# mabdullahsoyturk/Torch-Sputnik

Measured on AMD Instinct MI355X. Metric: SpMM effective GFLOP/s (2*nnz*N/t), M=N=K=4096 fp32, density 0.1, higher is better.
Workload: dtype f32

## Files before the change

torch_sputnik_amd/csrc/gen_spmm_flat.py:

```python
#!/usr/bin/env python3
import argparse

_ap = argparse.ArgumentParser()
_ap.add_argument("--mode", default="entry", choices=["entry", "group"])
_ap.add_argument("--layout", default="straight", choices=["straight", "diagonal"])
_ap.add_argument("out", nargs="?")
ARGS = _ap.parse_args()
GROUP = ARGS.mode == "group"

BK = 32
BK_SHIFT = 5
ROW_BYTES = 2048
ROW_SHIFT = 11
WIN_BYTES = 144
NSTRIP = 4
NPIECES = 4
ROWSTEP = 8

V_LANE, V_STAGE, V_PLAN, V_ROWS = "v0", "v1", "v2", "v3"
CUR_OFF, CUR_VAL = 4, 5
NXT_OFF, NXT_VAL, NXT_ROWS = 6, 7, 8
NN_OFF, NN_VAL, NN_ROWS = 10, 11, 12
PAIR = [16, 18, 20, 22]
VALT = [16, 18]
V_ADDR = 20
STRIP = [32, 40, 48, 56]
ACC = 64

S_STREAM, S_VALUES, S_CINFO, S_DENSE = "s[36:37]", "s[38:39]", "s[40:41]", "s[42:43]"
S_PITCH, S_KMAX, S_NCHUNKS, S_ROW0, S_LDS0, S_DEBUG = "s44", "s45", "s46", "s47", "s48", "s49"
S_REM, S_C, S_CIOFF, S_MINE, S_SB, S_NSW = "s50", "s51", "s56", "s57", "s76", "s77"
S_CI = ["s52", "s53", "s54", "s55"]
S_RET, S_BND = "s[58:59]", "s[60:61]"
S_ROWS = [62, 63, 64, 65]
S_IDX = [66, 67, 68, 69]
S_COLS = "s78"
S_T = ["s70", "s71", "s72", "s73", "s74", "s75"]

out = []


def emit(line):
    out.append(line)


def label(name):
    return f".L_{name}_%="


def strip_reads(ring, addr):
    s = STRIP[ring]
    emit(f"ds_read_b128 v[{s}:{s + 3}], v{addr}")
    emit(f"ds_read_b128 v[{s + 4}:{s + 7}], v{addr} offset:1024")


def fmas(src_pair, op_sel, ring):
    s = STRIP[ring]
    for q in range(4):
        emit(f"v_pk_fma_f32 v[{ACC + 2 * q}:{ACC + 2 * q + 1}], v[{src_pair}:{src_pair + 1}], "
             f"v[{s + 2 * q}:{s + 2 * q + 1}], v[{ACC + 2 * q}:{ACC + 2 * q + 1}] {op_sel}")


def entry_fma_stage(ring, lgkm):
    emit(f"s_waitcnt lgkmcnt({lgkm})")
    emit(f"s_set_gpr_idx_on s{S_IDX[ring]}, 0xc")
    fmas(PAIR[ring], "op_sel:[1,0,0] op_sel_hi:[1,1,1]", ring)
    emit("s_set_gpr_idx_off")


def entry_slot(slot):
    ring = slot % NSTRIP
    p = PAIR[ring]
    emit(f"{label(f'E_{slot}')}:")
    emit(f"s_sub_u32 {S_REM}, {S_REM}, 1")
    emit(f"s_cbranch_scc1 {label(f'bnd_{slot}')}")
    emit(f"v_mov_b64_dpp v[{p}:{p + 1}], v[{CUR_OFF}:{CUR_VAL}] row_newbcast:{slot} row_mask:0xf bank_mask:0xf")
    emit(f"s_bfe_u32 s{S_IDX[ring]}, s{S_ROWS[slot // 4]}, {hex(8 * (slot % 4) | (7 << 16))}")
    emit(f"v_add_u32 v{p}, v{p}, {V_LANE}")
    strip_reads(ring, p)
    entry_fma_stage((ring + 1) % NSTRIP, 2 * (NSTRIP - 1))


def group_entry_body(ring, slot):
    t = VALT[slot % 2]
    emit(f"v_mov_b32_dpp v{t}, v{CUR_VAL} row_newbcast:{slot} row_mask:0xf bank_mask:0xf")
    emit(f"s_bfe_u32 s{S_IDX[0]}, s{S_ROWS[slot // 4]}, {hex(8 * (slot % 4) | (7 << 16))}")
    emit(f"s_set_gpr_idx_on s{S_IDX[0]}, 0xc")
    fmas(t, "op_sel:[0,0,0] op_sel_hi:[0,1,1]", ring)
    emit("s_set_gpr_idx_off")


def group_start(ring, slot):
    emit(f"{label(f'N_{ring}_{slot}')}:")
    emit(f"s_sub_u32 {S_REM}, {S_REM}, 1")
    emit(f"s_cbranch_scc1 {label(f'bnd_{slot}')}")
    emit(f"v_mov_b32_dpp v{V_ADDR}, v{CUR_OFF} row_newbcast:{slot} row_mask:0xf bank_mask:0xf")
    emit(f"v_add_u32 v{V_ADDR}, v{V_ADDR}, {V_LANE}")
    strip_reads(ring, V_ADDR)
    emit(f"s_waitcnt lgkmcnt({2 * (NSTRIP - 1)})")


def first_groups():
    for i in range(NSTRIP - 1):
        emit(f"s_bfe_u32 {S_T[0]}, {S_COLS}, {hex(8 * i | (8 << 16))}")
        emit(f"s_lshl_b32 {S_T[0]}, {S_T[0]}, {ROW_SHIFT}")
        emit(f"v_add_u32 v{V_ADDR}, {S_T[0]}, {V_LANE}")
        strip_reads(i, V_ADDR)


def stage_chunk(chunk_sgpr):
    t_row, t_lds, t_r, t_lo, t_hi = S_T[1], S_T[2], S_T[3], S_T[4], S_T[5]
    emit(f"s_lshl_b32 {t_row}, {chunk_sgpr}, {BK_SHIFT}")
    emit(f"s_add_u32 {t_row}, {t_row}, {S_ROW0}")
    emit(f"s_and_b32 {t_lds}, {chunk_sgpr}, 1")
    emit(f"s_lshl_b32 {t_lds}, {t_lds}, 16")
    emit(f"s_add_u32 {t_lds}, {t_lds}, {S_LDS0}")
    for i in range(NPIECES):
        emit(f"s_add_u32 {t_r}, {t_row}, {ROWSTEP * i}")
        emit(f"s_min_u32 {t_r}, {t_r}, {S_KMAX}")
        emit(f"s_mul_hi_u32 {t_hi}, {t_r}, {S_PITCH}")
        emit(f"s_mul_i32 {t_lo}, {t_r}, {S_PITCH}")
        emit(f"s_add_u32 {t_lo}, {t_lo}, s42")
        emit(f"s_addc_u32 {t_hi}, {t_hi}, s43")
        emit(f"s_add_u32 m0, {t_lds}, {hex(ROWSTEP * i * ROW_BYTES)}")
        emit("s_nop 0")
        emit(f"global_load_lds_dwordx4 {V_STAGE}, s[{t_lo[1:]}:{t_hi[1:]}]")


def plan_load(off, rows):
    emit(f"global_load_dwordx2 v[{off}:{off + 1}], {V_PLAN}, {S_STREAM}")
    emit(f"global_load_dword v{rows}, {V_ROWS}, {S_STREAM}")
    emit(f"v_add_u32 {V_PLAN}, {hex(WIN_BYTES)}, {V_PLAN}")
    emit(f"v_add_u32 {V_ROWS}, {hex(WIN_BYTES)}, {V_ROWS}")


def gather(val):
    emit(f"global_load_dword v{val}, v{val}, {S_VALUES}")


def switch_window(tag):
    emit(f"s_cmp_lg_u32 {S_SB}, 0")
    emit(f"s_cbranch_scc1 {label('swc_' + tag)}")
    emit("s_waitcnt vmcnt(0)")
    emit(f"s_branch {label('swd_' + tag)}")
    emit(f"{label('swc_' + tag)}:")
    emit(f"s_waitcnt vmcnt({NPIECES})")
    emit(f"{label('swd_' + tag)}:")
    emit(f"s_mov_b32 {S_SB}, 0")
    emit(f"s_add_u32 {S_NSW}, {S_NSW}, 1")
    for i in range(4):
        emit(f"v_readlane_b32 s{S_ROWS[i]}, v{NXT_ROWS}, {i}")
    emit(f"v_bfe_u32 v{CUR_OFF}, v{NXT_OFF}, {8 if GROUP else 0}, 8")
    emit(f"v_mov_b32 v{CUR_VAL}, v{NXT_VAL}")
    emit(f"v_lshlrev_b32 v{CUR_OFF}, {ROW_SHIFT}, v{CUR_OFF}")
    emit(f"v_mov_b64 v[{NXT_OFF}:{NXT_VAL}], v[{NN_OFF}:{NN_VAL}]")
    emit(f"v_mov_b32 v{NXT_ROWS}, v{NN_ROWS}")
    emit(f"s_bitcmp1_b32 {S_DEBUG}, 3")
    emit(f"s_cbranch_scc1 {label('swskip_' + tag)}")
    gather(NXT_VAL)
    plan_load(NN_OFF, NN_ROWS)
    emit(f"{label('swskip_' + tag)}:")
    emit("s_nop 1")


def take_chunk_info():
    emit(f"s_mov_b32 {S_REM}, {S_CI[0] if GROUP else S_CI[3]}")
    if GROUP:
        emit(f"s_mov_b32 {S_COLS}, {S_CI[1]}")


def generate():
    emit("; ---- prologue ----")
    for r in list(range(ACC, ACC + 64)) + list(range(STRIP[0], STRIP[0] + 32)) + list(range(16, 24)):
        emit(f"v_mov_b32 v{r}, 0")
    for r in S_IDX:
        emit(f"s_mov_b32 s{r}, 0")
    emit(f"s_getpc_b64 {S_BND}")
    emit(f"{label('pc')}:")
    emit(f"s_add_u32 s60, s60, {label('boundary')}-{label('pc')}")
    emit("s_addc_u32 s61, s61, 0")
    plan_load(NXT_OFF, NXT_ROWS)
    plan_load(NN_OFF, NN_ROWS)
    emit("s_waitcnt vmcnt(2)")
    gather(NXT_VAL)
    emit(f"s_mov_b32 {S_T[0]}, 0")
    stage_chunk(S_T[0])
    emit(f"s_load_dwordx4 s[52:55], {S_CINFO}, 0x0")
    emit("s_waitcnt vmcnt(0) lgkmcnt(0)")
    emit("s_barrier")
    take_chunk_info()
    emit(f"s_load_dwordx4 s[52:55], {S_CINFO}, 0x10")
    emit(f"s_mov_b32 {S_CIOFF}, 32")
    emit(f"s_mov_b32 {S_C}, 0")
    emit(f"s_mov_b32 {S_NSW}, 0")
    emit(f"s_mov_b32 {S_SB}, 0")
    emit(f"s_mov_b32 {S_MINE}, 0")
    if GROUP:
        first_groups()
    emit(f"s_cmp_lt_u32 {S_NCHUNKS}, 2")
    emit(f"s_cbranch_scc1 {label('pro_nostage')}")
    emit(f"s_mov_b32 {S_T[0]}, 1")
    stage_chunk(S_T[0])
    emit(f"s_mov_b32 {S_SB}, 1")
    emit(f"s_mov_b32 {S_MINE}, 1")
    emit(f"{label('pro_nostage')}:")
    switch_window("pro")

    emit("; ---- main loop ----")
    if not GROUP:
        for slot in range(16):
            entry_slot(slot)
        switch_window("w")
        emit(f"s_branch {label('E_0')}")
    elif ARGS.layout == "straight":
        emit(f"s_branch {label(f'E_{NSTRIP - 1}_0')}")
        for ring in range(NSTRIP):
            for slot in range(16):
                emit(f"{label(f'E_{ring}_{slot}')}:")
                emit(f"s_bitcmp1_b32 s{S_ROWS[slot // 4]}, {8 * (slot % 4) + 7}")
                emit(f"s_cbranch_scc1 {label(f'N_{ring}_{slot}')}")
                emit(f"{label(f'B_{ring}_{slot}')}:")
                group_entry_body(ring, slot)
            switch_window(f"r{ring}")
            emit(f"s_branch {label(f'E_{ring}_0')}")
        emit("; ---- first entry of a column group ----")
        for ring in range(NSTRIP):
            for slot in range(16):
                group_start(ring, slot)
                emit(f"s_branch {label(f'B_{(ring + 1) % NSTRIP}_{slot}')}")
    else:
        emit(f"s_branch {label(f'E_{NSTRIP - 1}_0')}")
        for diag in range(NSTRIP):
            for slot in range(16):
                ring = (diag + slot) % NSTRIP
                emit(f"{label(f'E_{ring}_{slot}')}:")
                emit(f"s_bitcmp1_b32 s{S_ROWS[slot // 4]}, {8 * (slot % 4) + 7}")
                emit(f"s_cbranch_scc0 {label(f'B_{ring}_{slot}')}")
                group_start(ring, slot)
                emit(f"{label(f'B_{(ring + 1) % NSTRIP}_{slot}')}:")
                group_entry_body((ring + 1) % NSTRIP, slot)
            ring = (diag + 16) % NSTRIP
            switch_window(f"r{diag}")
            emit(f"s_branch {label(f'E_{ring}_0')}")

    emit("; ---- boundary stubs ----")
    for slot in range(16):
        emit(f"{label(f'bnd_{slot}')}:")
        emit(f"s_swappc_b64 {S_RET}, {S_BND}")
        if GROUP:
            emit(f"s_cbranch_scc1 {label('end')}")
            emit(f"s_branch {label(f'N_{NSTRIP - 1}_{slot}')}")
        else:
            emit(f"s_cbranch_scc1 {label(f'drain_{slot % NSTRIP}')}")
            emit(f"s_branch {label(f'E_{slot}')}")

    emit("; ---- boundary subroutine ----")
    emit(f"{label('boundary')}:")
    emit(f"s_bitcmp1_b32 {S_DEBUG}, 2")
    emit(f"s_cbranch_scc1 {label('bnodrain')}")
    emit("s_waitcnt lgkmcnt(0)")
    emit(f"{label('bnodrain')}:")
    emit(f"s_cmp_eq_u32 {S_MINE}, 0")
    emit(f"s_cbranch_scc1 {label('bvd')}")
    emit(f"s_bitcmp1_b32 {S_DEBUG}, 5")
    emit(f"s_cbranch_scc1 {label('bvd')}")
    for n in range(3):
        emit(f"s_cmp_eq_u32 {S_NSW}, {n}")
        emit(f"s_cbranch_scc1 {label(f'bv{n}')}")
    emit("s_waitcnt vmcnt(9)")
    emit(f"s_branch {label('bvd')}")
    for n in range(3):
        emit(f"{label(f'bv{n}')}:")
        emit(f"s_waitcnt vmcnt({3 * n})")
        if n < 2:
            emit(f"s_branch {label('bvd')}")
    emit(f"{label('bvd')}:")
    emit(f"s_bitcmp1_b32 {S_DEBUG}, 1")
    emit(f"s_cbranch_scc1 {label('bnobar')}")
    emit("s_barrier")
    emit(f"{label('bnobar')}:")
    emit(f"s_add_u32 {S_C}, {S_C}, 1")
    emit(f"s_cmp_eq_u32 {S_C}, {S_NCHUNKS}")
    emit(f"s_cbranch_scc1 {label('bret')}")
    take_chunk_info()
    emit(f"s_load_dwordx4 s[52:55], {S_CINFO}, {S_CIOFF}")
    emit(f"s_add_u32 {S_CIOFF}, {S_CIOFF}, 16")
    if GROUP:
        first_groups()
    emit(f"s_mov_b32 {S_NSW}, 0")
    emit(f"s_mov_b32 {S_MINE}, 0")
    emit(f"s_add_u32 {S_T[0]}, {S_C}, 1")
    emit(f"s_cmp_ge_u32 {S_T[0]}, {S_NCHUNKS}")
    emit(f"s_cbranch_scc1 {label('bnostage')}")
    emit(f"s_bitcmp1_b32 {S_DEBUG}, 0")
    emit(f"s_cbranch_scc1 {label('bnostage')}")
    stage_chunk(S_T[0])
    emit(f"s_add_u32 {S_SB}, {S_SB}, 1")
    emit(f"s_mov_b32 {S_MINE}, 1")
    emit(f"{label('bnostage')}:")
    emit(f"s_cmp_eq_u32 {S_C}, {S_NCHUNKS}")
    emit(f"{label('bret')}:")
    emit(f"s_setpc_b64 {S_RET}")

    if not GROUP:
        emit("; ---- drain: the three entries still in the pipeline ----")
        for ring in range(NSTRIP):
            emit(f"{label(f'drain_{ring}')}:")
            for j in range(1, NSTRIP):
                entry_fma_stage((ring + j) % NSTRIP, 2 * (NSTRIP - 1 - j))
            if ring < NSTRIP - 1:
                emit(f"s_branch {label('end')}")
    emit(f"{label('end')}:")
    emit("s_waitcnt vmcnt(0) lgkmcnt(0)")


def main():
    generate()
    text = "// GENERATED by gen_spmm_flat.py -- do not edit.\n" + "".join(
        f'"{line}\\n"\n' for line in out)
    if ARGS.out:
        with open(ARGS.out, "w") as f:
            f.write(text)
    else:
        print(text, end="")


if __name__ == "__main__":
    main()
```

torch_sputnik_amd/csrc/spmm_flat.hip:

```cpp
#include <algorithm>

#include "options.h"
#include "spmm_tiled_common.h"

namespace sputnik_hip {

namespace {

using namespace tiled;

constexpr int kBN = 512;
constexpr int kBK = 32;
constexpr int kWaves = 16;
constexpr int kRPW = 8;
constexpr int kBM = kWaves * kRPW;
constexpr int kAhead = 3;
constexpr int kDealPer = 256;
constexpr int kWindow = 16;
constexpr int kWindowBytes = 144;
constexpr int kTailWindows = 4;
constexpr int kMaxColumns = 65536;
constexpr unsigned kNewGroup = 0x80;


struct ChunkInfo {
  int groups;
  unsigned first_rows;
  unsigned unused;
  int entries;
};

__host__ __device__ inline size_t fill_tables_bytes(int nchunks) {
  return (sizeof(int) * (static_cast<size_t>(nchunks) * (kBK / 4 + 4) + 2 * kRPW + 2) + 15) / 16 * 16;
}
__device__ __forceinline__ int wave_sum(int v) {
#pragma unroll
  for (int o = 32; o > 0; o >>= 1) v += __shfl_xor(v, o);
  return v;
}
__device__ __forceinline__ int wave_inclusive_scan(int v, int lane) {
#pragma unroll
  for (int o = 1; o < 64; o <<= 1) {
    const int t = __shfl_up(v, o);
    if (lane >= o) v += t;
  }
  return v;
}

__global__ __launch_bounds__(kRPW * 64) void spmm_flat_fill_kernel(
    int m, int k, int slots, int nchunks, const int* __restrict__ row_indices,
    const int* __restrict__ row_offsets, const int* __restrict__ column_indices,
    int* __restrict__ row_ok, ChunkInfo* __restrict__ cinfo, int* __restrict__ gwin,
    unsigned char* __restrict__ stream, int stage_windows, int debug) {
  extern __shared__ unsigned lds[];
  constexpr int RPW = kRPW, BK = kBK, NT = RPW * 64;
  constexpr int WPC = BK / 4;
  constexpr int UN = 4;
  const int g = blockIdx.x, tid = threadIdx.x, lane = tid % 64, wave = tid / 64;
  const int groups = gridDim.x;
  unsigned* maskw = lds;
  int* ebase = reinterpret_cast<int*>(lds + nchunks * WPC);
  unsigned* nzmask = reinterpret_cast<unsigned*>(ebase + nchunks);
  unsigned* wprefix = nzmask + nchunks;
  int* scratch = reinterpret_cast<int*>(wprefix + 2 * nchunks);
  unsigned char* sbuf = reinterpret_cast<unsigned char*>(lds) + fill_tables_bytes(nchunks);

  for (int i = tid; i < nchunks * WPC; i += NT) maskw[i] = 0;
  const int slot = g * RPW + wave;
  const int entry = dealt_index(slot, slots, kDealPer);
  int p0 = 0, p1 = 0;
  if (entry < m) {
    const int row = row_indices[entry];
    p0 = row_offsets[row];
    p1 = row_offsets[row + 1];
  }
  int before = 0;
  for (int gp = tid; gp < g; gp += NT) {
    int rows[RPW], len = 0;
    int2 bounds[RPW];
#pragma unroll
    for (int r = 0; r < RPW; ++r) {
      const int e = dealt_index(gp * RPW + r, slots, kDealPer);
      rows[r] = e < m ? row_indices[e] : -1;
    }
#pragma unroll
    for (int r = 0; r < RPW; ++r) {
      typedef int int2_a4 __attribute__((ext_vector_type(2), aligned(4)));
      if (rows[r] >= 0) {
        const int2_a4 pair = *reinterpret_cast<const int2_a4*>(row_offsets + rows[r]);
        bounds[r] = make_int2(pair.x, pair.y);
      } else {
        bounds[r] = make_int2(0, 0);
      }
    }
#pragma unroll
    for (int r = 0; r < RPW; ++r) len += bounds[r].y - bounds[r].x;
    before += (len + kWindow - 1) / kWindow;
  }
  before = wave_sum(before);
  if (lane == 0) {
    scratch[wave] = before;
    scratch[RPW + wave] = p1 - p0;
  }
  if (tid == 0) scratch[2 * RPW] = 1;
  __syncthreads();
  int wbase = 0, total = 0;
#pragma unroll
  for (int r = 0; r < RPW; ++r) {
    wbase += scratch[r];
    total += scratch[RPW + r];
  }
  if (tid == 0) gwin[g] = wbase;
  unsigned char* my_stream = stream + static_cast<int64_t>(wbase) * kWindowBytes;
  const int windows = (total + kWindow - 1) / kWindow;

  bool ok = true;
  for (int base = p0; base < p1; base += 64 * UN) {
    int cur[UN], prev[UN];
#pragma unroll
    for (int u = 0; u < UN; ++u) {
      const int p = base + u * 64 + lane;
      cur[u] = p < p1 ? column_indices[p] : -2;
    }
    const int before_base = base > p0 ? column_indices[base - 1] : -1;
#pragma unroll
    for (int u = 0; u < UN; ++u) {
      const int up = __shfl_up(cur[u], 1);
      const int carry = u == 0 ? before_base : __shfl(cur[u == 0 ? 0 : u - 1], 63);
      prev[u] = lane == 0 ? carry : up;
    }
#pragma unroll
    for (int u = 0; u < UN; ++u) {
      if (cur[u] == -2) continue;
      if (cur[u] <= prev[u] || cur[u] >= k) ok = false;
      else atomicOr(&maskw[cur[u] >> 2], (1u << wave) << (8 * (cur[u] & 3)));
    }
  }
  const bool wave_ok = __builtin_amdgcn_ballot_w64(!ok) == 0;
  if (lane == 0) {
    row_ok[slot] = wave_ok ? 1 : 0;
    if (!wave_ok) scratch[2 * RPW] = 0;
  }
  __syncthreads();
  ChunkInfo* my_info = cinfo + static_cast<int64_t>(g) * (nchunks + 1);
  if (scratch[2 * RPW] == 0) {
    unsigned* w = reinterpret_cast<unsigned*>(my_stream);
    const int nwin = windows + (g == groups - 1 ? kTailWindows : 0);
    for (int i = tid; i < nwin * (kWindowBytes / 4); i += NT)
      w[i] = i % (kWindowBytes / 4) >= 32 ? 0x80808080u : 0u;
    for (int c = tid; c <= nchunks; c += NT) my_info[c] = ChunkInfo{0, 0u, 0u, 0};
    return;
  }

  if (debug & 0x100) return;
  for (int t0 = 0; t0 < nchunks * WPC; t0 += NT) {
    const int t = t0 + tid;
    const bool live = t < nchunks * WPC;
    const int c = t / WPC, i = t % WPC;
    const unsigned w = live ? maskw[t] : 0u;
    const int cnt = __popc(w);
    unsigned nz = 0u;
#pragma unroll
    for (int b = 0; b < 4; ++b)
      if ((w >> (8 * b)) & 0xffu) nz |= 1u << (4 * i + b);
    int incl = cnt;
#pragma unroll
    for (int o = 1; o < WPC; o <<= 1) {
      const int up = __shfl_up(incl, o, WPC);
      if (i >= o) incl += up;
    }
#pragma unroll
    for (int o = 1; o < WPC; o <<= 1) nz |= static_cast<unsigned>(__shfl_xor(static_cast<int>(nz), o, WPC));
    const int entries = __shfl(incl, WPC - 1, WPC);
    if (live) {
      reinterpret_cast<unsigned char*>(wprefix)[t] = static_cast<unsigned char>(incl - cnt);
      if (i == 0) {
        unsigned first = 0u, rest = nz;
        const int cgroups = __popc(nz);
#pragma unroll
        for (int q = 0; q < kAhead; ++q)
          if (rest) {
            first |= static_cast<unsigned>((c & 1) * BK + __ffs(rest) - 1) << (8 * q);
            rest &= rest - 1u;
          }
        ebase[c] = entries;
        nzmask[c] = nz;
        my_info[c] = ChunkInfo{cgroups, first, 0u, entries};
      }
    }
  }
  if (tid == 0) my_info[nchunks] = ChunkInfo{0, 0u, 0u, 0};
  __syncthreads();
  if (wave == 0) {
    int carry = 0;
    for (int c0 = 0; c0 < nchunks; c0 += 64) {
      const int c = c0 + lane;
      const int e = c < nchunks ? ebase[c] : 0;
      const int incl = wave_inclusive_scan(e, lane);
      if (c < nchunks) ebase[c] = carry + incl - e;
      carry += __shfl(incl, 63);
    }
  }
  __syncthreads();

  if (debug & 0x200) return;
  static_assert(WPC == 8, "two prefix words per chunk");
  const int nwin_out = windows + (g == groups - 1 ? kTailWindows : 0);
  const bool staged = nwin_out <= stage_windows && !(debug & 0x1000);
  unsigned char* const dst_stream = staged ? sbuf : my_stream;
  for (int base = p0; base < p1; base += 64 * UN) {
    int cols[UN];
#pragma unroll
    for (int u = 0; u < UN; ++u) {
      const int p = base + u * 64 + lane;
      cols[u] = p < p1 ? column_indices[p] : -1;
    }
#pragma unroll
    for (int u = 0; u < UN; ++u) {
      if (cols[u] < 0) continue;
      const int p = base + u * 64 + lane;
      const int col = cols[u], c = col / BK, j = col % BK;
      const unsigned w = maskw[c * WPC + j / 4];
      const int prefix = static_cast<int>((wprefix[2 * c + j / 16] >> (8 * ((j / 4) % 4))) & 0xffu) +
                         __popc(w & ((1u << (8 * (j & 3))) - 1u));
      const unsigned byte = (w >> (8 * (j & 3))) & 0xffu;
      const int own = __popc(byte & ((1u << wave) - 1u));
      const int pos = ebase[c] + prefix + own;
      unsigned rowbyte = wave * 8, tile_rows = static_cast<unsigned>((c & 1) * BK + j);
      if (own == 0) {
        rowbyte |= kNewGroup;
        unsigned ahead = j == BK - 1 ? 0u : nzmask[c] >> (j + 1);
        ahead &= ahead - 1u;
        ahead &= ahead - 1u;
        if (ahead) tile_rows |= static_cast<unsigned>((c & 1) * BK + j + __ffs(ahead)) << 8;
      }
      if (debug & 0x400) continue;
      unsigned char* block = dst_stream + static_cast<int64_t>(pos / kWindow) * kWindowBytes;
      const int e = pos % kWindow;
      *reinterpret_cast<uint2*>(block + 8 * e) = make_uint2(tile_rows, static_cast<unsigned>(p) * 4u);
      block[128 + e] = static_cast<unsigned char>(rowbyte);
    }
  }
  for (int pos = total + tid; pos < windows * kWindow; pos += NT) {
    unsigned char* block = dst_stream + static_cast<int64_t>(pos / kWindow) * kWindowBytes;
    *reinterpret_cast<uint2*>(block + 8 * (pos % kWindow)) = make_uint2(0u, 0u);
    block[128 + pos % kWindow] = static_cast<unsigned char>(kNewGroup);
  }
  if (g == groups - 1) {
    unsigned* w = reinterpret_cast<unsigned*>(dst_stream + static_cast<int64_t>(windows) * kWindowBytes);
    for (int i = tid; i < kTailWindows * (kWindowBytes / 4); i += NT)
      w[i] = i % (kWindowBytes / 4) >= 32 ? 0x80808080u : 0u;
  }
  if (staged) {
    __syncthreads();
    const uint4* src = reinterpret_cast<const uint4*>(sbuf);
    uint4* dst = reinterpret_cast<uint4*>(my_stream);
    for (int i = tid; i < nwin_out * (kWindowBytes / 16); i += NT) dst[i] = src[i];
  }
}

using v8f = float __attribute__((ext_vector_type(8)));

#define SPUTNIK_HIP_FLAT_ASM_OPERANDS                                                              \
      : "={v[64:71]}"(a0), "={v[72:79]}"(a1), "={v[80:87]}"(a2), "={v[88:95]}"(a3),                \
        "={v[96:103]}"(a4), "={v[104:111]}"(a5), "={v[112:119]}"(a6), "={v[120:127]}"(a7)          \
      : "{v0}"(lane_base), "{v1}"(stage_off), "{v2}"(plan_off), "{v3}"(rows_off),                  \
        "{s[36:37]}"(my_stream), "{s[38:39]}"(values), "{s[40:41]}"(my_info), "{s[42:43]}"(dense), \
        "{s44}"(pitch), "{s45}"(kmax), "{s46}"(nchunks), "{s47}"(row0), "{s48}"(lds0),             \
        "{s49}"(debug)                                                                             \
      : "memory", "m0", "scc", "v4", "v5", "v6", "v7", "v8", "v9", "v10", "v11", "v12", "v13",     \
        "v14", "v15", "v16", "v17", "v18", "v19", "v20", "v21", "v22", "v23", "v32", "v33", "v34", \
        "v35", "v36", "v37", "v38", "v39", "v40", "v41", "v42", "v43", "v44", "v45", "v46", "v47", \
        "v48", "v49", "v50", "v51", "v52", "v53", "v54", "v55", "v56", "v57", "v58", "v59", "v60", \
        "v61", "v62", "v63", "s50", "s51", "s52", "s53", "s54", "s55", "s56", "s57", "s58", "s59", \
        "s60", "s61", "s62", "s63", "s64", "s65", "s66", "s67", "s68", "s69", "s70", "s71", "s72", \
        "s73", "s74", "s75", "s76", "s77", "s78", "s79", "s80"

template <int LOOP>
__global__ __launch_bounds__(kWaves * 64) void spmm_flat_kernel(
    int m, int k, int n, int slots, int nchunks, int n_tiles, const int* __restrict__ row_indices,
    const float* __restrict__ values, int64_t values_stride, const ChunkInfo* __restrict__ cinfo,
    const int* __restrict__ gwin, const unsigned char* __restrict__ stream,
    const float* __restrict__ dense, int64_t dense_stride, float* __restrict__ out,
    int64_t out_stride, const int* __restrict__ row_ok, const int* __restrict__ row_offsets,
    const int* __restrict__ column_indices, int debug, Epilogue epi) {
  constexpr int RPW = kRPW, BM = kBM, BN = kBN, BK = kBK, VEC = 8;
  constexpr int PPR = VEC / 4;
  __shared__ float tile[2][BK * BN];

  const int lane = threadIdx.x % kWave;
  const int wave = __builtin_amdgcn_readfirstlane(threadIdx.x / kWave);

  const int bid = blockIdx.x;
  int ntile, mblock;
  int replica = blockIdx.y;
  const int xcd_cols = 1 << ((debug >> 13) & 3);
  if (xcd_cols > 1 && n_tiles == 8 && (gridDim.x / 8) % xcd_cols == 0) {
    const int xcd = bid % 8, i = bid / 8, col_groups = 8 / xcd_cols;
    ntile = (xcd % col_groups) * xcd_cols + i % xcd_cols;
    mblock = (xcd / col_groups) * ((gridDim.x / 8) / xcd_cols) + i / xcd_cols;
  } else if (n_tiles % 8 == 0) {
    const int per_xcd = n_tiles / 8;
    const int xcd = bid % 8, i = bid / 8;
    ntile = xcd * per_xcd + i % per_xcd;
    mblock = i / per_xcd;
  } else {
    const int work = xcd_local_index32();
    const int mblocks = gridDim.x / n_tiles;
    mblock = work % mblocks;
    ntile = (work / mblocks) % n_tiles;
    replica = work / (mblocks * n_tiles);
  }
  values += replica * values_stride;
  dense += replica * dense_stride;
  out += replica * out_stride;

  const int n0 = ntile * BN;
  const int slot0 = mblock * BM + wave * RPW;

  if (!block_rows_ok_wave(row_ok, mblock * BM, BM)) {
    for (int r = 0; r < RPW; ++r) {
      const int entry = dealt_index(slot0 + r, slots, kDealPer);
      if (entry >= m) continue;
      const int row = row_indices[entry];
#pragma unroll
      for (int h = 0; h < PPR; ++h) {
        if (n0 + h * 256 + lane * 4 >= n) continue;
        const int col = min(n0 + h * 256 + lane * 4, n - 4);
        const float4 acc4 = gather_row_strip(values, column_indices, row_offsets[row],
                                             row_offsets[row + 1], dense + col, n);
        *reinterpret_cast<float4*>(out + static_cast<int64_t>(row) * n + col) =
            apply_epilogue(acc4, epi, row);
      }
    }
    return;
  }

  const int group = slot0 / RPW;
  const unsigned char* my_stream =
      stream + static_cast<int64_t>(__builtin_amdgcn_readfirstlane(gwin[group])) * kWindowBytes;
  const ChunkInfo* my_info = cinfo + static_cast<int64_t>(group) * (nchunks + 1);
  const unsigned tile_lds = static_cast<unsigned>(reinterpret_cast<uintptr_t>(AS_LDS(&tile[0][0])));
  const unsigned lane_base = tile_lds + lane * 16;
  const unsigned stage_off =
      static_cast<unsigned>(min(n0 + (wave % PPR) * 256 + lane * 4, n - 4)) * 4u;
  const unsigned plan_off = (lane & 15) * 8, rows_off = 128 + (lane & 3) * 4;
  const int pitch = n * 4, kmax = k - 1, row0 = wave / PPR;
  const int lds0 = static_cast<int>(tile_lds) + (wave / PPR) * (BN * 4) + (wave % PPR) * 1024;

  v8f a0, a1, a2, a3, a4, a5, a6, a7;
  if constexpr (LOOP == 0) {
    asm volatile(
#include "spmm_flat_body_entry.inc"
        SPUTNIK_HIP_FLAT_ASM_OPERANDS);
  } else if constexpr (LOOP == 1) {
    asm volatile(
#include "spmm_flat_body_group_s.inc"
        SPUTNIK_HIP_FLAT_ASM_OPERANDS);
  } else {
    asm volatile(
#include "spmm_flat_body_group_d.inc"
        SPUTNIK_HIP_FLAT_ASM_OPERANDS);
  }

  const v8f acc[8] = {a0, a1, a2, a3, a4, a5, a6, a7};
#pragma unroll
  for (int r = 0; r < RPW; ++r) {
    const int entry = dealt_index(slot0 + r, slots, kDealPer);
    if (entry < m) {
      const int row = row_indices[entry];
#pragma unroll
      for (int h = 0; h < PPR; ++h)
        if (n0 + h * 256 + lane * 4 < n) {
          const int col = min(n0 + h * 256 + lane * 4, n - 4);
          const int f = r * VEC + 4 * h;
          *reinterpret_cast<float4*>(out + static_cast<int64_t>(row) * n + col) =
              apply_epilogue(make_float4(acc[f / 8][f % 8], acc[f / 8][f % 8 + 1],
                                         acc[f / 8][f % 8 + 2], acc[f / 8][f % 8 + 3]),
                             epi, row);
        }
    }
  }
}

struct FlatPlan {
  int slots, nchunks, n_tiles, groups;
  size_t row_ok_off, cinfo_off, gwin_off, stream_off, bytes;
};

FlatPlan make_flat_plan(int m, int k, int n, int nonzeros) {
  FlatPlan p;
  p.slots = ceil_div(m, kDealPer) * kDealPer;
  p.nchunks = ceil_div(k, kBK);
  p.n_tiles = ceil_div(n, kBN);
  p.groups = p.slots / kRPW;
  auto up = [](size_t v) { return (v + 255) / 256 * 256; };
  p.row_ok_off = 0;
  p.cinfo_off = row_ok_bytes(p.slots);
  p.gwin_off = up(p.cinfo_off + sizeof(ChunkInfo) * static_cast<size_t>(p.nchunks + 1) * p.groups);
  p.stream_off = up(p.gwin_off + sizeof(int) * static_cast<size_t>(p.groups));
  const size_t windows = static_cast<size_t>(nonzeros) / kWindow + p.groups + kTailWindows;
  p.bytes = up(p.stream_off + windows * kWindowBytes);
  return p;
}

int fill_stage_windows(int nchunks, int nonzeros, int groups) {
  const size_t tables = fill_tables_bytes(nchunks);
  if (tables + kWindowBytes > 64 * 1024) return 0;
  const int64_t room = static_cast<int64_t>((64 * 1024 - tables) / kWindowBytes);
  const int64_t want = (static_cast<int64_t>(nonzeros) / kWindow / groups) * 5 / 4 + kTailWindows + 2;
  return static_cast<int>(std::min(room, want));
}
size_t fill_lds_bytes(int nchunks, int stage_windows) {
  return fill_tables_bytes(nchunks) + static_cast<size_t>(stage_windows) * kWindowBytes;
}

int flat_mode(int m, int k, int nonzeros) {
  const int forced = options().spmm_sparse;
  if (forced >= 2 && forced <= 4) return forced - 2;
  const double d = static_cast<double>(nonzeros) / (static_cast<double>(m) * k);
  return d < 0.12 ? 0 : d < 0.36 ? 2 : 1;
}

}

static bool fill_lds_available(int k) {
  static const bool extended = [] {
    return hipFuncSetAttribute(reinterpret_cast<const void*>(spmm_flat_fill_kernel),
                               hipFuncAttributeMaxDynamicSharedMemorySize,
                               static_cast<int>(fill_lds_bytes(kMaxColumns / kBK, 0))) == hipSuccess;
  }();
  return extended || fill_lds_bytes(ceil_div(k, kBK), 0) <= 64 * 1024;
}

bool spmm_flat_applicable(int m, int k, int n, int nonzeros) {
  if (n < 4 || k < kBK || m < 64 || nonzeros < 16 * static_cast<int64_t>(m) ||
      nonzeros >= (1 << 29))
    return false;
  if (static_cast<int64_t>(ceil_div(n, kBN)) * kBN * 3 > static_cast<int64_t>(n) * 4) return false;
  return k <= kMaxColumns && m <= 16384 && fill_lds_available(k);
}

const char* spmm_flat_kernel_name(int m, int k, int nonzeros) {
  static const char* const names[] = {"spmm_flat_kernel<0>", "spmm_flat_kernel<1>", "spmm_flat_kernel<2>"};
  return names[flat_mode(m, k, nonzeros)];
}

int64_t spmm_flat_tiles(int m, int n) {
  return static_cast<int64_t>(ceil_div(m, kBM)) * ceil_div(n, kBN);
}

size_t spmm_flat_workspace_bytes(int m, int k, int n, int nonzeros) {
  return make_flat_plan(m, k, n, nonzeros).bytes;
}

int spmm_flat_plan(int m, int k, int n, int nonzeros, const int* row_indices,
                   const int* row_offsets, const int* column_indices, void* workspace,
                   hipStream_t stream) {
  const FlatPlan p = make_flat_plan(m, k, n, nonzeros);
  char* base = static_cast<char*>(workspace);
  if (!fill_lds_available(k)) return SPUTNIK_HIP_UNSUPPORTED;
  const int stage_windows = fill_stage_windows(p.nchunks, nonzeros, p.groups);
  hipLaunchKernelGGL(spmm_flat_fill_kernel, dim3(p.groups), dim3(kRPW * 64),
                     fill_lds_bytes(p.nchunks, stage_windows), stream, m, k, p.slots, p.nchunks, row_indices,
                     row_offsets, column_indices, reinterpret_cast<int*>(base + p.row_ok_off),
                     reinterpret_cast<ChunkInfo*>(base + p.cinfo_off),
                     reinterpret_cast<int*>(base + p.gwin_off),
                     reinterpret_cast<unsigned char*>(base + p.stream_off), stage_windows,
                     options().spmm_debug);
  return launch_status();
}

int xcd_columns_code(int k, int n, int nonzeros, int row_blocks) {
  const int forced = options().spmm_debug;
  if (forced & 0x8000) return (forced >> 13) & 3;
  if (ceil_div(n, kBN) != 8) return 0;
  const double stream = 13.0 * nonzeros, b = 4.0 * k * n;
  int best = 0;
  double best_bytes = stream * 8 + b;
  for (int code = 1; code <= 3; ++code) {
    const int c = 1 << code;
    if (row_blocks % c != 0) break;
    const double bytes = stream * 8 / c + b * c;
    if (bytes < 0.97 * best_bytes) {
      best = code;
      best_bytes = bytes;
    }
  }
  return best;
}

int spmm_flat_exec(int m, int k, int n, int nonzeros, int replicas, const int* row_indices,
                   const float* values, int64_t values_stride, const int* row_offsets,
                   const int* column_indices, const float* dense, int64_t dense_stride, float* out,
                   int64_t out_stride, const void* workspace, hipStream_t stream, Epilogue epi) {
  const FlatPlan p = make_flat_plan(m, k, n, nonzeros);
  const char* base = static_cast<const char*>(workspace);
#define SPUTNIK_HIP_LAUNCH_FLAT(LOOP)                                                              \
  hipLaunchKernelGGL((spmm_flat_kernel<LOOP>), dim3((p.slots / kBM) * p.n_tiles, replicas),        \
                     dim3(kWaves * 64), 0, stream, m, k, n, p.slots, p.nchunks, p.n_tiles,         \
                     row_indices, values, values_stride,                                           \
                     reinterpret_cast<const ChunkInfo*>(base + p.cinfo_off),                       \
                     reinterpret_cast<const int*>(base + p.gwin_off),                              \
                     reinterpret_cast<const unsigned char*>(base + p.stream_off), dense,           \
                     dense_stride, out, out_stride,                                                \
                     reinterpret_cast<const int*>(base + p.row_ok_off), row_offsets,               \
                     column_indices, debug_word, epi)
  const int debug_word = (options().spmm_debug & ~0xe000) |
                         (xcd_columns_code(k, n, nonzeros, p.slots / kBM) << 13);
  switch (flat_mode(m, k, nonzeros)) {
    case 0: SPUTNIK_HIP_LAUNCH_FLAT(0); break;
    case 1: SPUTNIK_HIP_LAUNCH_FLAT(1); break;
    default: SPUTNIK_HIP_LAUNCH_FLAT(2); break;
  }
#undef SPUTNIK_HIP_LAUNCH_FLAT
  return launch_status();
}

}
```

Before: 42760.

## Overlap prologue loads with setup in SpMM plan build and main kernel

In the plan-building kernel, the row-index, row-offset and first column-index loads are issued together before the window-count loop. The first two rounds of column indices are kept in registers so the placement pass reuses them instead of reloading. The main kernel now issues the first chunk's dense-row LDS DMA, the row_ok check, the gwin read and the row-index loads before the validity branch, and hoists the plan loads in the generated assembly prologue. The intent is to hide global-memory latency in the prologues, at the cost of more live registers and a speculative DMA on the fallback path. Debug bits are added to skip the main loop or the epilogue.

```diff
diff --git a/torch_sputnik_amd/csrc/gen_spmm_flat.py b/torch_sputnik_amd/csrc/gen_spmm_flat.py
--- a/torch_sputnik_amd/csrc/gen_spmm_flat.py
+++ b/torch_sputnik_amd/csrc/gen_spmm_flat.py
@@ -171,6 +171,9 @@
 
 def generate():
     emit("; ---- prologue ----")
+    plan_load(NXT_OFF, NXT_ROWS)
+    plan_load(NN_OFF, NN_ROWS)
+    emit(f"s_load_dwordx4 s[52:55], {S_CINFO}, 0x0")
     for r in list(range(ACC, ACC + 64)) + list(range(STRIP[0], STRIP[0] + 32)) + list(range(16, 24)):
         emit(f"v_mov_b32 v{r}, 0")
     for r in S_IDX:
@@ -179,13 +182,8 @@
     emit(f"{label('pc')}:")
     emit(f"s_add_u32 s60, s60, {label('boundary')}-{label('pc')}")
     emit("s_addc_u32 s61, s61, 0")
-    plan_load(NXT_OFF, NXT_ROWS)
-    plan_load(NN_OFF, NN_ROWS)
     emit("s_waitcnt vmcnt(2)")
     gather(NXT_VAL)
-    emit(f"s_mov_b32 {S_T[0]}, 0")
-    stage_chunk(S_T[0])
-    emit(f"s_load_dwordx4 s[52:55], {S_CINFO}, 0x0")
     emit("s_waitcnt vmcnt(0) lgkmcnt(0)")
     emit("s_barrier")
     take_chunk_info()
@@ -205,6 +203,8 @@
     emit(f"s_mov_b32 {S_MINE}, 1")
     emit(f"{label('pro_nostage')}:")
     switch_window("pro")
+    emit(f"s_bitcmp1_b32 {S_DEBUG}, 6")
+    emit(f"s_cbranch_scc1 {label('end')}")
 
     emit("; ---- main loop ----")
     if not GROUP:
diff --git a/torch_sputnik_amd/csrc/spmm_flat.hip b/torch_sputnik_amd/csrc/spmm_flat.hip
--- a/torch_sputnik_amd/csrc/spmm_flat.hip
+++ b/torch_sputnik_amd/csrc/spmm_flat.hip
@@ -66,43 +66,94 @@
   unsigned char* sbuf = reinterpret_cast<unsigned char*>(lds) + fill_tables_bytes(nchunks);
 
   for (int i = tid; i < nchunks * WPC; i += NT) maskw[i] = 0;
+  if (tid == 0) scratch[2 * RPW] = 1;
+  typedef int int2_a4 __attribute__((ext_vector_type(2), aligned(4)));
   const int slot = g * RPW + wave;
   const int entry = dealt_index(slot, slots, kDealPer);
+  auto load_rows = [&](int gp, int (&rows)[RPW]) {
+#pragma unroll
+    for (int r = 0; r < RPW; ++r)
+      rows[r] = row_indices[min(dealt_index(gp * RPW + r, slots, kDealPer), m - 1)];
+  };
+  auto load_bounds = [&](const int (&rows)[RPW], int2_a4 (&bounds)[RPW]) {
+#pragma unroll
+    for (int r = 0; r < RPW; ++r) bounds[r] = *reinterpret_cast<const int2_a4*>(row_offsets + rows[r]);
+  };
+  auto windows_of = [&](int gp, const int2_a4 (&bounds)[RPW]) {
+    int len = 0;
+#pragma unroll
+    for (int r = 0; r < RPW; ++r)
+      if (dealt_index(gp * RPW + r, slots, kDealPer) < m) len += bounds[r].y - bounds[r].x;
+    return (len + kWindow - 1) / kWindow;
+  };
   int p0 = 0, p1 = 0;
-  if (entry < m) {
-    const int row = row_indices[entry];
-    p0 = row_offsets[row];
-    p1 = row_offsets[row + 1];
-  }
+  auto load_round = [&](int base, int (&cols)[UN]) {
+#pragma unroll
+    for (int u = 0; u < UN; ++u) {
+      const int p = base + u * 64 + lane;
+      cols[u] = p < p1 ? column_indices[p] : -2;
+    }
+  };
+  int kept0[UN], kept1[UN];
   int before = 0;
-  for (int gp = tid; gp < g; gp += NT) {
-    int rows[RPW], len = 0;
-    int2 bounds[RPW];
-#pragma unroll
-    for (int r = 0; r < RPW; ++r) {
-      const int e = dealt_index(gp * RPW + r, slots, kDealPer);
-      rows[r] = e < m ? row_indices[e] : -1;
-    }
-#pragma unroll
-    for (int r = 0; r < RPW; ++r) {
-      typedef int int2_a4 __attribute__((ext_vector_type(2), aligned(4)));
-      if (rows[r] >= 0) {
-        const int2_a4 pair = *reinterpret_cast<const int2_a4*>(row_offsets + rows[r]);
-        bounds[r] = make_int2(pair.x, pair.y);
-      } else {
-        bounds[r] = make_int2(0, 0);
-      }
-    }
-#pragma unroll
-    for (int r = 0; r < RPW; ++r) len += bounds[r].y - bounds[r].x;
-    before += (len + kWindow - 1) / kWindow;
-  }
+  {
+    const int gp = tid < g ? tid : 0;
+    int rows[RPW];
+    int2_a4 bounds[RPW];
+    const int row = row_indices[min(entry, m - 1)];
+    load_rows(gp, rows);
+    const int2_a4 own = *reinterpret_cast<const int2_a4*>(row_offsets + row);
+    load_bounds(rows, bounds);
+    if (entry < m) p0 = own.x, p1 = own.y;
+    load_round(p0, kept0);
+    __syncthreads();
+    if (tid < g) before = windows_of(gp, bounds);
+  }
+  for (int gp = tid + NT; gp < g; gp += NT) {
+    int rows[RPW];
+    int2_a4 bounds[RPW];
+    load_rows(gp, rows);
+    load_bounds(rows, bounds);
+    before += windows_of(gp, bounds);
+  }
+
+  bool ok = true;
+  auto check_round = [&](const int (&cur)[UN], int before_base) {
+    int prev[UN];
+#pragma unroll
+    for (int u = 0; u < UN; ++u) {
+      const int up = __shfl_up(cur[u], 1);
+      const int carry = u == 0 ? before_base : __shfl(cur[u == 0 ? 0 : u - 1], 63);
+      prev[u] = lane == 0 ? carry : up;
+    }
+#pragma unroll
+    for (int u = 0; u < UN; ++u) {
+      if (cur[u] == -2) continue;
+      if (cur[u] <= prev[u] || cur[u] >= k) ok = false;
+      else atomicOr(&maskw[cur[u] >> 2], (1u << wave) << (8 * (cur[u] & 3)));
+    }
+  };
+  check_round(kept0, -1);
+  if (p1 - p0 > 64 * UN) {
+    load_round(p0 + 64 * UN, kept1);
+    check_round(kept1, __shfl(kept0[UN - 1], 63));
+  } else {
+#pragma unroll
+    for (int u = 0; u < UN; ++u) kept1[u] = -2;
+  }
+  for (int base = p0 + 2 * 64 * UN; base < p1; base += 64 * UN) {
+    int cur[UN];
+    load_round(base, cur);
+    check_round(cur, column_indices[base - 1]);
+  }
+  const bool wave_ok = __builtin_amdgcn_ballot_w64(!ok) == 0;
   before = wave_sum(before);
   if (lane == 0) {
     scratch[wave] = before;
     scratch[RPW + wave] = p1 - p0;
-  }
-  if (tid == 0) scratch[2 * RPW] = 1;
+    row_ok[slot] = wave_ok ? 1 : 0;
+    if (!wave_ok) scratch[2 * RPW] = 0;
+  }
   __syncthreads();
   int wbase = 0, total = 0;
 #pragma unroll
@@ -113,35 +164,6 @@
   if (tid == 0) gwin[g] = wbase;
   unsigned char* my_stream = stream + static_cast<int64_t>(wbase) * kWindowBytes;
   const int windows = (total + kWindow - 1) / kWindow;
-
-  bool ok = true;
-  for (int base = p0; base < p1; base += 64 * UN) {
-    int cur[UN], prev[UN];
-#pragma unroll
-    for (int u = 0; u < UN; ++u) {
-      const int p = base + u * 64 + lane;
-      cur[u] = p < p1 ? column_indices[p] : -2;
-    }
-    const int before_base = base > p0 ? column_indices[base - 1] : -1;
-#pragma unroll
-    for (int u = 0; u < UN; ++u) {
-      const int up = __shfl_up(cur[u], 1);
-      const int carry = u == 0 ? before_base : __shfl(cur[u == 0 ? 0 : u - 1], 63);
-      prev[u] = lane == 0 ? carry : up;
-    }
-#pragma unroll
-    for (int u = 0; u < UN; ++u) {
-      if (cur[u] == -2) continue;
-      if (cur[u] <= prev[u] || cur[u] >= k) ok = false;
-      else atomicOr(&maskw[cur[u] >> 2], (1u << wave) << (8 * (cur[u] & 3)));
-    }
-  }
-  const bool wave_ok = __builtin_amdgcn_ballot_w64(!ok) == 0;
-  if (lane == 0) {
-    row_ok[slot] = wave_ok ? 1 : 0;
-    if (!wave_ok) scratch[2 * RPW] = 0;
-  }
-  __syncthreads();
   ChunkInfo* my_info = cinfo + static_cast<int64_t>(g) * (nchunks + 1);
   if (scratch[2 * RPW] == 0) {
     unsigned* w = reinterpret_cast<unsigned*>(my_stream);
@@ -208,13 +230,7 @@
   const int nwin_out = windows + (g == groups - 1 ? kTailWindows : 0);
   const bool staged = nwin_out <= stage_windows && !(debug & 0x1000);
   unsigned char* const dst_stream = staged ? sbuf : my_stream;
-  for (int base = p0; base < p1; base += 64 * UN) {
-    int cols[UN];
-#pragma unroll
-    for (int u = 0; u < UN; ++u) {
-      const int p = base + u * 64 + lane;
-      cols[u] = p < p1 ? column_indices[p] : -1;
-    }
+  auto place_round = [&](int base, const int (&cols)[UN]) {
 #pragma unroll
     for (int u = 0; u < UN; ++u) {
       if (cols[u] < 0) continue;
@@ -240,6 +256,13 @@
       *reinterpret_cast<uint2*>(block + 8 * e) = make_uint2(tile_rows, static_cast<unsigned>(p) * 4u);
       block[128 + e] = static_cast<unsigned char>(rowbyte);
     }
+  };
+  place_round(p0, kept0);
+  place_round(p0 + 64 * UN, kept1);
+  for (int base = p0 + 2 * 64 * UN; base < p1; base += 64 * UN) {
+    int cols[UN];
+    load_round(base, cols);
+    place_round(base, cols);
   }
   for (int pos = total + tid; pos < windows * kWindow; pos += NT) {
     unsigned char* block = dst_stream + static_cast<int64_t>(pos / kWindow) * kWindowBytes;
@@ -318,7 +341,27 @@
   const int n0 = ntile * BN;
   const int slot0 = mblock * BM + wave * RPW;
 
-  if (!block_rows_ok_wave(row_ok, mblock * BM, BM)) {
+  const unsigned stage_off =
+      static_cast<unsigned>(min(n0 + (wave % PPR) * 256 + lane * 4, n - 4)) * 4u;
+  const int kmax = k - 1, row0 = wave / PPR;
+  float* const first_piece = &tile[0][0] + row0 * BN + (wave % PPR) * 256;
+#pragma unroll
+  for (int i = 0; i < BK * PPR / kWaves; ++i)
+    lds_dma_row(dense + static_cast<int64_t>(min(row0 + (kWaves / PPR) * i, kmax)) * n, stage_off,
+                first_piece + (kWaves / PPR) * i * BN);
+  static_assert(BM == 2 * kWave, "two row_ok words per lane");
+  const int ok_words = row_ok[mblock * BM + lane] & row_ok[mblock * BM + kWave + lane];
+  const int group = slot0 / RPW;
+  const int first_window = gwin[group];
+  int rows[RPW];
+#pragma unroll
+  for (int r = 0; r < RPW; ++r) {
+    const int entry = dealt_index(slot0 + r, slots, kDealPer);
+    rows[r] = entry < m ? row_indices[entry] : -1;
+  }
+
+  if (__builtin_amdgcn_ballot_w64(ok_words == 0) != 0) {
+    wait_vm<0>();
     for (int r = 0; r < RPW; ++r) {
       const int entry = dealt_index(slot0 + r, slots, kDealPer);
       if (entry >= m) continue;
@@ -336,16 +379,13 @@
     return;
   }
 
-  const int group = slot0 / RPW;
   const unsigned char* my_stream =
-      stream + static_cast<int64_t>(__builtin_amdgcn_readfirstlane(gwin[group])) * kWindowBytes;
+      stream + static_cast<int64_t>(__builtin_amdgcn_readfirstlane(first_window)) * kWindowBytes;
   const ChunkInfo* my_info = cinfo + static_cast<int64_t>(group) * (nchunks + 1);
   const unsigned tile_lds = static_cast<unsigned>(reinterpret_cast<uintptr_t>(AS_LDS(&tile[0][0])));
   const unsigned lane_base = tile_lds + lane * 16;
-  const unsigned stage_off =
-      static_cast<unsigned>(min(n0 + (wave % PPR) * 256 + lane * 4, n - 4)) * 4u;
   const unsigned plan_off = (lane & 15) * 8, rows_off = 128 + (lane & 3) * 4;
-  const int pitch = n * 4, kmax = k - 1, row0 = wave / PPR;
+  const int pitch = n * 4;
   const int lds0 = static_cast<int>(tile_lds) + (wave / PPR) * (BN * 4) + (wave % PPR) * 1024;
 
   v8f a0, a1, a2, a3, a4, a5, a6, a7;
@@ -363,12 +403,12 @@
         SPUTNIK_HIP_FLAT_ASM_OPERANDS);
   }
 
+  if (debug & 0x10) return;
   const v8f acc[8] = {a0, a1, a2, a3, a4, a5, a6, a7};
 #pragma unroll
   for (int r = 0; r < RPW; ++r) {
-    const int entry = dealt_index(slot0 + r, slots, kDealPer);
-    if (entry < m) {
-      const int row = row_indices[entry];
+    const int row = rows[r];
+    if (row >= 0) {
 #pragma unroll
       for (int h = 0; h < PPR; ++h)
         if (n0 + h * 256 + lane * 4 < n) {
```

Result: no change. 42800 (median of 2 runs) (+0.1%).
